# mikelodder7/bls-bn254

Hardware: AMD Instinct MI355X
Metric: BN254 pairings/sec (= BLS verifies/sec) (higher is better)
Workload: dtype int64; 1 GPU; 262144 batched single-sig BLS verifies per GPU (BASELINE configs[1]), unique 32-byte messages, 1024-key pool, 1/64 invalid tuples; key de-duplication + hash-to-G1 + per-key G2 checks and line tables + 2-pair Miller loop + final exp; tuples_per_gpu=262144, tuples_total=262144, key_pool=1024

## Files before the change

### bls-bn254_amd/csrc/pairing.h

```cpp
#pragma once
#include "curve.h"

namespace bn {

struct G2J { Fp2 x, y, z; };
struct Line { Fp2 c0, c1, c2; };

BN_FUNC Line doubling_step(G2J& r) {
  BN_CTX;
  Fp2 tmp0 = fp2_sqr(r.x);
  Fp2 tmp1 = fp2_sqr(r.y);
  Fp2 tmp2 = fp2_sqr(tmp1);
  Fp2 s3 = fp2_sqr(fp2_norm(fp2_add(tmp1, r.x)));
  Fp2 tmp3 = f_lc3<2, -2, -2>(s3, tmp0, tmp2);
  Fp2 tmp4 = f_lc2<3, 0>(tmp0, tmp0);
  Fp2 tmp6 = fp2_norm(fp2_add(r.x, tmp4));
  Fp2 tmp5 = fp2_sqr(tmp4);
  Fp2 zsq = fp2_sqr(r.z);
  Fp2 nx = f_lc2<1, -2>(tmp5, tmp3);
  Fp2 nz = fp2_norm(fp2_sub(fp2_sub(fp2_sqr(fp2_norm(fp2_add(r.z, r.y))), tmp1), zsq));
  Fp2 ny = f_lc2<1, -8>(fp2_mul(fp2_sub(tmp3, nx), tmp4), tmp2);
  Line l;
  l.c1 = f_lc2<-2, 0>(fp2_mul(tmp4, zsq), zsq);
  Fp2 s6 = fp2_sub(fp2_sub(fp2_sqr(tmp6), tmp0), tmp5);
  l.c2 = f_lc2<1, -4>(s6, tmp1);
  l.c0 = f_lc2<2, 0>(fp2_mul(nz, zsq), zsq);
  r.x = nx; r.y = ny; r.z = nz;
  return l;
}
BN_FUNC Line addition_step(G2J& r, const Fp2& qx, const Fp2& qy) {
  BN_CTX;
  Fp2 zsq = fp2_sqr(r.z);
  Fp2 ysq = fp2_sqr(qy);
  Fp2 t0 = fp2_mul(zsq, qx);
  Fp2 sy = fp2_sqr(fp2_norm(fp2_add(qy, r.z)));
  Fp2 t1 = fp2_mul(fp2_norm(fp2_sub(fp2_sub(sy, ysq), zsq)), zsq);
  Fp2 t2 = fp2_norm(fp2_sub(t0, r.x));
  Fp2 t3 = fp2_sqr(t2);
  Fp2 t4 = f_lc2<4, 0>(t3, t3);
  Fp2 t5 = fp2_mul(t4, t2);
  Fp2 t6 = f_lc2<1, -2>(t1, r.y);
  Fp2 t9 = fp2_mul(t6, qx);
  Fp2 t7 = fp2_mul(t4, r.x);
  Fp2 nx = f_lc3<1, -1, -2>(fp2_sqr(t6), t5, t7);
  Fp2 nz = fp2_norm(fp2_sub(fp2_sub(fp2_sqr(fp2_norm(fp2_add(r.z, t2))), zsq), t3));
  Fp2 t8 = fp2_mul(fp2_sub(t7, nx), t6);
  Fp2 ny = f_lc2<1, -2>(t8, fp2_mul(r.y, t5));
  Fp2 s10 = fp2_sqr(fp2_norm(fp2_add(qy, nz)));
  Fp2 t10 = fp2_sub(fp2_sub(s10, ysq), fp2_sqr(nz));
  Line l;
  l.c2 = f_lc2<2, -1>(t9, t10);
  l.c0 = f_lc2<2, 0>(nz, nz);
  l.c1 = f_lc2<-2, 0>(t6, t6);
  r.x = nx; r.y = ny; r.z = nz;
  return l;
}
BN_FUNC Fp12 ell(const Fp12& f, const Line& l, const Fp& px, const Fp& py) {
  BN_CTX;
  return fp12_mul_by_034(f, fp2_mul_fp(l.c0, py), fp2_mul_fp(l.c1, px), l.c2);
}
BN_FUNC Fp12 ell2(const Fp12& f, const Line& la, const Fp& pax, const Fp& pay, const Line& lb, const Fp& pbx, const Fp& pby) {
  BN_CTX;
  return fp12_mul_by_two_lines(f, fp2_mul_fp(la.c0, pay), fp2_mul_fp(la.c1, pax), la.c2, fp2_mul_fp(lb.c0, pby), fp2_mul_fp(lb.c1, pbx), lb.c2);
}
BN_INL Line fp2_norm_line(const Line& l) { return {fp2_norm(l.c0), fp2_norm(l.c1), fp2_norm(l.c2)}; }
BN_INL Line line_from_table(const int32_t* t) {
  return {fp2_from_limbs(t), fp2_from_limbs(t + 18), fp2_from_limbs(t + 36)};
}

constexpr uint64_t ate_naf_mask(int word, bool neg) {
  uint64_t m = 0;
  for (int i = 0; i < 64; ++i) {
    int j = 64 * word + i;
    if (j < bnc::ATE_NAF_LEN && (neg ? bnc::ATE_NAF[j] < 0 : bnc::ATE_NAF[j] != 0)) m |= (uint64_t)1 << i;
  }
  return m;
}
BN_INL int ate_naf_digit(int j) {
  constexpr uint64_t nz0 = ate_naf_mask(0, false), nz1 = ate_naf_mask(1, false), ng0 = ate_naf_mask(0, true), ng1 = ate_naf_mask(1, true);
  const uint64_t nz = j < 64 ? nz0 : nz1, ng = j < 64 ? ng0 : ng1;
  const int b = j & 63;
  return ((nz >> b) & 1) ? (((ng >> b) & 1) ? -1 : 1) : 0;
}
BN_FUNC Fp12 miller_loop_1(const G1A& p, const G2A& q) {
  BN_CTX;
  Fp12 f = fp12_one();
  G2J T = {q.x, q.y, fp2_one()};
  Fp2 nqy = fp2_norm(fp2_neg(q.y));
  for (int j = bnc::ATE_NAF_LEN - 2; j >= 0; --j) {
    f = fp12_sqr(f);
    f = ell(f, doubling_step(T), p.x, p.y);
    int d = ate_naf_digit(j);
    if (d != 0) f = ell(f, addition_step(T, q.x, d > 0 ? q.y : nqy), p.x, p.y);
  }
  Fp2 g2 = fp2_const(bnc::GAMMA1[1]), g3 = fp2_const(bnc::GAMMA1[2]);
  Fp2 q1x = fp2_mul(fp2_norm(fp2_conj(q.x)), g2), q1y = fp2_mul(fp2_norm(fp2_conj(q.y)), g3);
  Fp2 q2x = fp2_mul(fp2_norm(fp2_conj(q1x)), g2);
  Fp2 q2y = fp2_norm(fp2_neg(fp2_mul(fp2_norm(fp2_conj(q1y)), g3)));
  f = ell(f, addition_step(T, q1x, q1y), p.x, p.y);
  f = ell(f, addition_step(T, q2x, q2y), p.x, p.y);
  return f;
}

BN_FUNC Fp12 miller_loop_verify(const G1A& sig, const G1A& h, const G2A& pk,
                                     const int32_t (*table)[54]) {
  BN_CTX;
  Fp12 f = fp12_one();
  G2J T = {pk.x, pk.y, fp2_one()};
  Fp2 nqy = fp2_norm(fp2_neg(pk.y));
  int ti = 0;
  for (int j = bnc::ATE_NAF_LEN - 2; j >= 0; --j) {
    f = fp12_sqr(f);
    f = ell(f, line_from_table(table[ti++]), sig.x, sig.y);
    f = ell(f, doubling_step(T), h.x, h.y);
    int d = ate_naf_digit(j);
    if (d != 0) {
      f = ell(f, line_from_table(table[ti++]), sig.x, sig.y);
      f = ell(f, addition_step(T, pk.x, d > 0 ? pk.y : nqy), h.x, h.y);
    }
  }
  Fp2 g2 = fp2_const(bnc::GAMMA1[1]), g3 = fp2_const(bnc::GAMMA1[2]);
  Fp2 q1x = fp2_mul(fp2_norm(fp2_conj(pk.x)), g2), q1y = fp2_mul(fp2_norm(fp2_conj(pk.y)), g3);
  Fp2 q2x = fp2_mul(fp2_norm(fp2_conj(q1x)), g2);
  Fp2 q2y = fp2_norm(fp2_neg(fp2_mul(fp2_norm(fp2_conj(q1y)), g3)));
  f = ell(f, line_from_table(table[ti++]), sig.x, sig.y);
  f = ell(f, addition_step(T, q1x, q1y), h.x, h.y);
  f = ell(f, line_from_table(table[ti++]), sig.x, sig.y);
  f = ell(f, addition_step(T, q2x, q2y), h.x, h.y);
  return f;
}

BN_FUNC Fp12 miller_loop_verify_ws(const Ws& inv, const int32_t (*table)[54]) {
  Fp12 f = fp12_one();
  G2J T = {fp2_load_mem(ws_at(inv, 36)), fp2_load_mem(ws_at(inv, 54)), fp2_one()};
  int ti = 0;
  Ws p = inv;
  for (int j = bnc::ATE_NAF_LEN - 2; j >= 0; --j) {
    f = fp12_sqr(f);
    BN_OPAQUE(p);
    Fp sx = fp_load_mem(p), sy = fp_load_mem(ws_at(p, 9)), hx = fp_load_mem(ws_at(p, 18)), hy = fp_load_mem(ws_at(p, 27));
    BN_SCHED_BARRIER;
    Line l = doubling_step(T);
    f = ell2(f, line_from_table(table[ti++]), sx, sy, l, hx, hy);
    int d = ate_naf_digit(j);
    if (d != 0) {
      BN_OPAQUE(p);
      Fp2 qy = fp2_load_mem(ws_at(p, 54));
      Fp2 nqy = fp2_norm(fp2_neg(qy));
      Fp2 qx = fp2_load_mem(ws_at(p, 36));
      BN_OPAQUE(p);
      sx = fp_load_mem(p); sy = fp_load_mem(ws_at(p, 9)); hx = fp_load_mem(ws_at(p, 18)); hy = fp_load_mem(ws_at(p, 27));
      BN_SCHED_BARRIER;
      l = addition_step(T, qx, fp2_select(d > 0, qy, nqy));
      f = ell2(f, line_from_table(table[ti++]), sx, sy, l, hx, hy);
    }
  }
  BN_OPAQUE(p);
  Fp2 g2 = fp2_const(bnc::GAMMA1[1]), g3 = fp2_const(bnc::GAMMA1[2]);
  Fp2 q1x = fp2_mul(fp2_norm(fp2_conj(fp2_load_mem(ws_at(p, 36)))), g2);
  Fp2 q1y = fp2_mul(fp2_norm(fp2_conj(fp2_load_mem(ws_at(p, 54)))), g3);
  Fp2 q2x = fp2_mul(fp2_norm(fp2_conj(q1x)), g2);
  Fp2 q2y = fp2_norm(fp2_neg(fp2_mul(fp2_norm(fp2_conj(q1y)), g3)));
  Line l = addition_step(T, q1x, q1y);
  BN_OPAQUE(p);
  f = ell2(f, line_from_table(table[ti++]), fp_load_mem(p), fp_load_mem(ws_at(p, 9)), l, fp_load_mem(ws_at(p, 18)), fp_load_mem(ws_at(p, 27)));
  l = addition_step(T, q2x, q2y);
  BN_OPAQUE(p);
  f = ell2(f, line_from_table(table[ti++]), fp_load_mem(p), fp_load_mem(ws_at(p, 9)), l, fp_load_mem(ws_at(p, 18)), fp_load_mem(ws_at(p, 27)));
  return f;
}

BN_INL void g2j_store(const Ws& w, const G2J& t) { fp2_store_mem(w, t.x); fp2_store_mem(ws_at(w, 18), t.y); fp2_store_mem(ws_at(w, 36), t.z); }
BN_INL G2J g2j_load(const Ws& w) { return {fp2_load_mem(w), fp2_load_mem(ws_at(w, 18)), fp2_load_mem(ws_at(w, 36))}; }
BN_FUNC Fp12 miller_loop_verify_ws2(const Ws& inv, const Ws& park_in, const int32_t (*table)[54]) {
  Fp12 f = fp12_one();
  Ws p = inv, park = park_in;
  fp2_store_mem(park, fp2_load_mem(ws_at(inv, 36))); fp2_store_mem(ws_at(park, 18), fp2_load_mem(ws_at(inv, 54))); fp2_store_mem(ws_at(park, 36), fp2_one());
  BN_MEM_FENCE;
  int ti = 0;
  for (int j = bnc::ATE_NAF_LEN - 2; j >= 0; --j) {
    f = fp12_sqr(f);
    BN_OPAQUE(p); BN_OPAQUE(park);
    Fp sx = fp_load_mem(p), sy = fp_load_mem(ws_at(p, 9)), hx = fp_load_mem(ws_at(p, 18)), hy = fp_load_mem(ws_at(p, 27));
    G2J T = g2j_load(park);
    BN_SCHED_BARRIER;
    Line l = doubling_step(T);
    g2j_store(park, T);
    BN_MEM_FENCE;
    f = ell2(f, line_from_table(table[ti++]), sx, sy, l, hx, hy);
    int d = ate_naf_digit(j);
    if (d != 0) {
      BN_OPAQUE(p); BN_OPAQUE(park);
      Fp2 qy = fp2_load_mem(ws_at(p, 54));
      Fp2 nqy = fp2_norm(fp2_neg(qy));
      Fp2 qx = fp2_load_mem(ws_at(p, 36));
      sx = fp_load_mem(p); sy = fp_load_mem(ws_at(p, 9)); hx = fp_load_mem(ws_at(p, 18)); hy = fp_load_mem(ws_at(p, 27));
      T = g2j_load(park);
      BN_SCHED_BARRIER;
      l = addition_step(T, qx, fp2_select(d > 0, qy, nqy));
      g2j_store(park, T);
      BN_MEM_FENCE;
      f = ell2(f, line_from_table(table[ti++]), sx, sy, l, hx, hy);
    }
  }
  BN_OPAQUE(p); BN_OPAQUE(park);
  Fp2 g2 = fp2_const(bnc::GAMMA1[1]), g3 = fp2_const(bnc::GAMMA1[2]);
  Fp2 q1x = fp2_mul(fp2_norm(fp2_conj(fp2_load_mem(ws_at(p, 36)))), g2);
  Fp2 q1y = fp2_mul(fp2_norm(fp2_conj(fp2_load_mem(ws_at(p, 54)))), g3);
  Fp2 q2x = fp2_mul(fp2_norm(fp2_conj(q1x)), g2);
  Fp2 q2y = fp2_norm(fp2_neg(fp2_mul(fp2_norm(fp2_conj(q1y)), g3)));
  G2J T = g2j_load(park);
  Line l = addition_step(T, q1x, q1y);
  BN_OPAQUE(p);
  f = ell2(f, line_from_table(table[ti++]), fp_load_mem(p), fp_load_mem(ws_at(p, 9)), l, fp_load_mem(ws_at(p, 18)), fp_load_mem(ws_at(p, 27)));
  l = addition_step(T, q2x, q2y);
  BN_OPAQUE(p);
  f = ell2(f, line_from_table(table[ti++]), fp_load_mem(p), fp_load_mem(ws_at(p, 9)), l, fp_load_mem(ws_at(p, 18)), fp_load_mem(ws_at(p, 27)));
  return f;
}

BN_FUNC Fp12 miller_loop_1_ws(const Ws& inv_in, const Ws& park_in) {
  Fp12 f = fp12_one();
  Ws p = inv_in, park = park_in;
  fp2_store_mem(park, fp2_load_mem(ws_at(p, 18))); fp2_store_mem(ws_at(park, 18), fp2_load_mem(ws_at(p, 36))); fp2_store_mem(ws_at(park, 36), fp2_one());
  BN_MEM_FENCE;
  for (int j = bnc::ATE_NAF_LEN - 2; j >= 0; --j) {
    f = fp12_sqr(f);
    BN_OPAQUE(p); BN_OPAQUE(park);
    Fp px = fp_load_mem(p), py = fp_load_mem(ws_at(p, 9));
    G2J T = g2j_load(park);
    BN_SCHED_BARRIER;
    Line l = doubling_step(T);
    g2j_store(park, T);
    BN_MEM_FENCE;
    f = ell(f, l, px, py);
    int d = ate_naf_digit(j);
    if (d != 0) {
      BN_OPAQUE(p); BN_OPAQUE(park);
      Fp2 qy = fp2_load_mem(ws_at(p, 36));
      Fp2 nqy = fp2_norm(fp2_neg(qy));
      Fp2 qx = fp2_load_mem(ws_at(p, 18));
      px = fp_load_mem(p); py = fp_load_mem(ws_at(p, 9));
      T = g2j_load(park);
      BN_SCHED_BARRIER;
      l = addition_step(T, qx, fp2_select(d > 0, qy, nqy));
      g2j_store(park, T);
      BN_MEM_FENCE;
      f = ell(f, l, px, py);
    }
  }
  BN_OPAQUE(p); BN_OPAQUE(park);
  Fp2 g2 = fp2_const(bnc::GAMMA1[1]), g3 = fp2_const(bnc::GAMMA1[2]);
  Fp2 q1x = fp2_mul(fp2_norm(fp2_conj(fp2_load_mem(ws_at(p, 18)))), g2);
  Fp2 q1y = fp2_mul(fp2_norm(fp2_conj(fp2_load_mem(ws_at(p, 36)))), g3);
  Fp2 q2x = fp2_mul(fp2_norm(fp2_conj(q1x)), g2);
  Fp2 q2y = fp2_norm(fp2_neg(fp2_mul(fp2_norm(fp2_conj(q1y)), g3)));
  G2J T = g2j_load(park);
  Line l = addition_step(T, q1x, q1y);
  BN_OPAQUE(p);
  f = ell(f, l, fp_load_mem(p), fp_load_mem(ws_at(p, 9)));
  l = addition_step(T, q2x, q2y);
  BN_OPAQUE(p);
  f = ell(f, l, fp_load_mem(p), fp_load_mem(ws_at(p, 9)));
  return f;
}

BN_INL void line_store(const Ws& w, const Line& l) { fp2_store_mem(w, l.c0); fp2_store_mem(ws_at(w, 18), l.c1); fp2_store_mem(ws_at(w, 36), l.c2); }
BN_INL Line line_load(const Ws& w) { return {fp2_load_mem(w), fp2_load_mem(ws_at(w, 18)), fp2_load_mem(ws_at(w, 36))}; }
BN_INL Line line_mask(bool live, const Line& l) {
  return {fp2_select(live, l.c0, fp2_one()), fp2_select(live, l.c1, fp2_zero()), fp2_select(live, l.c2, fp2_zero())};
}
template <int KIND>
BN_FUNC Fp12 miller2_step(const Fp12& f_in, G2J& T, const Ws& park, const Ws& lpark, const Ws& hh_in, const Ws& qw_in, bool negq, bool live_a, bool live_b) {
  Ws hh = hh_in, qw = qw_in, pk = park, lp = lpark;
  BN_OPAQUE(hh); BN_OPAQUE(qw); BN_OPAQUE(pk); BN_OPAQUE(lp);
  const Fp2 g2 = fp2_const(bnc::GAMMA1[1]), g3 = fp2_const(bnc::GAMMA1[2]);
  auto q_of = [&](int pair, Fp2& qx, Fp2& qy) {
    qx = fp2_load_mem(ws_at(qw, 36 * pair)); qy = fp2_load_mem(ws_at(qw, 36 * pair + 18));
    if (KIND == 1) qy = fp2_select(negq, fp2_norm(fp2_neg(qy)), qy);
    if (KIND >= 2) { qx = fp2_mul(fp2_norm(fp2_conj(qx)), g2); qy = fp2_mul(fp2_norm(fp2_conj(qy)), g3); }
    if (KIND == 3) { qx = fp2_mul(fp2_norm(fp2_conj(qx)), g2); qy = fp2_norm(fp2_neg(fp2_mul(fp2_norm(fp2_conj(qy)), g3))); }
  };
  Line la;
  if (KIND == 0) la = doubling_step(T);
  else { Fp2 qx, qy; q_of(0, qx, qy); la = addition_step(T, qx, qy); }
  line_store(lp, fp2_norm_line(line_mask(live_a, la)));
  G2J Tb = g2j_load(pk);
  BN_MEM_FENCE;
  g2j_store(pk, T);
  BN_MEM_FENCE;
  Line lb;
  if (KIND == 0) lb = doubling_step(Tb);
  else { Fp2 qx, qy; q_of(1, qx, qy); lb = addition_step(Tb, qx, qy); }
  lb = line_mask(live_b, lb);
  T = g2j_load(pk);
  BN_MEM_FENCE;
  g2j_store(pk, Tb);
  BN_MEM_FENCE;
  la = line_load(lp);
  Fp hax = fp_load_mem(hh), hay = fp_load_mem(ws_at(hh, 9)), hbx = fp_load_mem(ws_at(hh, 18)), hby = fp_load_mem(ws_at(hh, 27));
  return ell2(f_in, la, hax, hay, lb, hbx, hby);
}
BN_FUNC Fp12 miller_loop_2var_ws(const Ws& hh, const Ws& qw, const Ws& park, const Ws& lpark, bool live_a, bool live_b) {
  Fp12 f = fp12_one();
  G2J T = {fp2_load_mem(qw), fp2_load_mem(ws_at(qw, 18)), fp2_one()};
  g2j_store(park, G2J{fp2_load_mem(ws_at(qw, 36)), fp2_load_mem(ws_at(qw, 54)), fp2_one()});
  BN_MEM_FENCE;
  for (int j = bnc::ATE_NAF_LEN - 2; j >= 0; --j) {
    f = fp12_sqr(f);
    f = miller2_step<0>(f, T, park, lpark, hh, qw, false, live_a, live_b);
    int d = ate_naf_digit(j);
    if (d != 0) f = miller2_step<1>(f, T, park, lpark, hh, qw, d < 0, live_a, live_b);
  }
  f = miller2_step<2>(f, T, park, lpark, hh, qw, false, live_a, live_b);
  f = miller2_step<3>(f, T, park, lpark, hh, qw, false, live_a, live_b);
  return f;
}

BN_FUNC Fp12 cyclotomic_exp_x(const Fp12& f) {
  BN_CTX;
  Fp12 r = f;
  for (int i = 61; i >= 0; --i) {
    r = fp12_cyclotomic_sqr(r);
    if ((bnc::BN_X >> i) & 1) r = fp12_mul(r, f);
  }
  return r;
}
BN_FUNC Fp12 cyclotomic_exp_x_chain(const Fp12& f, const Ws& slots, const Ws* park = nullptr) {
  const ChainOp prog[BN_X_CHAIN_LEN] = BN_X_CHAIN;
  fp12_store_mem(slots, f);
  BN_MEM_FENCE;
  Fp12 r = f;
  for (int k = 0; k < BN_X_CHAIN_LEN; ++k) {
    const ChainOp op = prog[k];
    if (op.load >= 0) r = fp12_load_mem(ws_at(slots, 108 * op.load));
    for (int q = 0; q < op.sq; ++q) r = fp12_cyclotomic_sqr(r);
    if (op.mul >= 0) r = fp12_mul_mem(r, ws_at(slots, 108 * op.mul), park);
    if (op.store >= 0) fp12_store_mem(ws_at(slots, 108 * op.store), r);
    if (op.cstore >= 0) { fp6_store_mem(ws_at(slots, 108 * op.cstore), r.c0); fp6_store_mem(ws_at(slots, 108 * op.cstore + 54), fp6_norm(fp6_neg(r.c1))); }
    if (op.store >= 0 || op.cstore >= 0) BN_MEM_FENCE;
  }
  return r;
}
BN_FUNC Fp12 fe_easy(const Fp12& f) {
  Fp12 t = fp12_mul(fp12_conj(f), fp12_inv(f));
  return fp12_mul(fp12_frob<2>(t), t);
}
struct FeEasyHead { Fp2 c0, c1, c2, nrm; Fp nu; };
BN_FUNC FeEasyHead fe_easy_head(const Fp12& a) {
  BN_CTX;
  Fp6 s0 = fp6_sqr(a.c0), s1 = fp6_sqr(a.c1);
  Fp6 d = {fp2_sub_mul_xi(s0.c0, s1.c2), fp2_norm(fp2_sub(s0.c1, s1.c0)), fp2_norm(fp2_sub(s0.c2, s1.c1))};
  Fp2 q0 = fp2_sqr(d.c0), q1 = fp2_sqr(d.c1), q2 = fp2_sqr(d.c2);
  Fp2 m01 = fp2_mul(d.c0, d.c1), m02 = fp2_mul(d.c0, d.c2), m12 = fp2_mul(d.c1, d.c2);
  FeEasyHead h;
  h.c0 = fp2_sub_mul_xi(q0, m12);
  h.c1 = fp2_norm(fp2_sub(fp2_mul_xi(q2), m01));
  h.c2 = fp2_norm(fp2_sub(q1, m02));
  Fp2 u = fp2_add(fp2_mul(d.c2, h.c1), fp2_mul(d.c1, h.c2));
  h.nrm = fp2_add_mul_xi(fp2_mul(d.c0, h.c0), u);
  h.nu = fp_dot2(h.nrm.c0, h.nrm.c0, h.nrm.c1, h.nrm.c1);
  return h;
}
BN_FUNC Fp12 fe_easy_tail(const Fp12& a, const FeEasyHead& h, const Fp& nu_inv) {
  BN_CTX;
  Fp2 ti = {fp_mul(h.nrm.c0, nu_inv), fp_mul(fp_neg(h.nrm.c1), nu_inv)};
  Fp6 t6 = {fp2_mul(h.c0, ti), fp2_mul(h.c1, ti), fp2_mul(h.c2, ti)};
  Fp12 inv = {fp6_mul(a.c0, t6), fp6_norm(fp6_neg(fp6_mul(a.c1, t6)))};
  Fp12 t = fp12_mul(fp12_conj(a), inv);
  return fp12_mul(fp12_frob<2>(t), t);
}
template <bool POW_FALLBACK = true>
BN_FUNC bool fp_inv4(Fp x[4]) {
  BN_CTX;
  bool z[4];
  Fp v[4], pre[4];
  for (int i = 0; i < 4; ++i) { z[i] = fp_is_zero(x[i]); v[i] = fp_select(z[i], fp_one(), fp_norm(x[i])); }
  pre[0] = v[0];
  for (int i = 1; i < 4; ++i) pre[i] = fp_mul(pre[i - 1], v[i]);
  bool done = true;
  Fp inv = POW_FALLBACK ? fp_inv(pre[3]) : fp_inv_divsteps(pre[3], done);
  for (int i = 3; i >= 1; --i) {
    Fp r = fp_mul(inv, pre[i - 1]);
    inv = fp_mul(inv, v[i]);
    x[i] = fp_select(z[i], fp_zero(), r);
  }
  x[0] = fp_select(z[0], fp_zero(), inv);
  return done;
}
BN_FUNC void fe_h1(const Fp12& x0, Fp12& a, Fp12& b) {
  a = fp12_cyclotomic_sqr(fp12_conj(x0));
  Fp12 a2 = fp12_cyclotomic_sqr(a);
  b = fp12_mul(a, a2);
}
BN_FUNC void fe_h2(const Fp12& x0, const Fp12& b, Fp12& c, Fp12& b2, Fp12& d2) {
  c = fp12_conj(x0);
  b2 = fp12_mul(c, fp12_conj(b));
  d2 = fp12_cyclotomic_sqr(c);
}
BN_FUNC Fp12 fe_h3(const Fp12& t, const Fp12& a, const Fp12& c, const Fp12& b2, const Fp12& x0) {
  Fp12 e = fp12_mul(b2, x0);
  Fp12 d = fp12_mul(a, e);
  Fp12 l0 = fp12_mul(t, fp12_mul(c, e));
  Fp12 r = fp12_mul(l0, fp12_frob<1>(d));
  r = fp12_mul(r, fp12_frob<2>(e));
  Fp12 l3 = fp12_mul(fp12_conj(t), d);
  return fp12_mul(r, fp12_frob<3>(l3));
}
BN_FUNC Fp12 final_exponentiation(const Fp12& f) {
  Fp12 t = fe_easy(f), a, b, c, b2, d2;
  fe_h1(cyclotomic_exp_x(t), a, b);
  fe_h2(cyclotomic_exp_x(b), b, c, b2, d2);
  return fe_h3(t, a, c, b2, cyclotomic_exp_x(d2));
}

BN_INL void fp2_to_be(uint8_t* out, const Fp2& c) { fp_to_be(out, c.c0); fp_to_be(out + 32, c.c1); }
BN_FUNC void fp12_to_be(uint8_t* out, const Fp12& a) {
  BN_CTX;
  fp2_to_be(out, a.c0.c0); fp2_to_be(out + 64, a.c0.c1); fp2_to_be(out + 128, a.c0.c2);
  fp2_to_be(out + 192, a.c1.c0); fp2_to_be(out + 256, a.c1.c1); fp2_to_be(out + 320, a.c1.c2);
}
BN_INL Fp2 fp2_from_be(const uint8_t* in, bool& ok) {
  bool o0, o1;
  Fp2 c = {fp_from_be(in, o0), fp_from_be(in + 32, o1)};
  ok &= o0 & o1;
  return c;
}
BN_FUNC Fp12 fp12_from_be(const uint8_t* in, bool& ok) {
  BN_CTX;
  ok = true;
  Fp12 a;
  a.c0.c0 = fp2_from_be(in, ok); a.c0.c1 = fp2_from_be(in + 64, ok); a.c0.c2 = fp2_from_be(in + 128, ok);
  a.c1.c0 = fp2_from_be(in + 192, ok); a.c1.c1 = fp2_from_be(in + 256, ok); a.c1.c2 = fp2_from_be(in + 320, ok);
  return a;
}
BN_INL void fp2_store_limbs(int32_t* out, size_t stride, const Fp2& c) {
  Fp c0 = fp_canon(c.c0), c1 = fp_canon(c.c1);
  BN_UNROLL for (int k = 0; k < NL; ++k) { out[(size_t)k * stride] = c0.l[k]; out[(size_t)(9 + k) * stride] = c1.l[k]; }
}
BN_INL void fp2_store_limbs(const Ws& w, const Fp2& c) {
  Fp c0 = fp_canon(c.c0), c1 = fp_canon(c.c1);
  BN_UNROLL for (int k = 0; k < NL; ++k) { ws_store(w, k, c0.l[k]); ws_store(w, 9 + k, c1.l[k]); }
}
BN_FUNC void fp12_store_limbs(const Ws& w, const Fp12& a) {
  BN_CTX;
  fp2_store_limbs(w, a.c0.c0); fp2_store_limbs(ws_at(w, 18), a.c0.c1); fp2_store_limbs(ws_at(w, 36), a.c0.c2);
  fp2_store_limbs(ws_at(w, 54), a.c1.c0); fp2_store_limbs(ws_at(w, 72), a.c1.c1); fp2_store_limbs(ws_at(w, 90), a.c1.c2);
}
BN_INL Fp2 fp2_load_limbs(const Ws& w) {
  Fp2 c;
  BN_UNROLL for (int k = 0; k < NL; ++k) { c.c0.l[k] = ws_load(w, k); c.c1.l[k] = ws_load(w, 9 + k); }
  BN_TRK(set_trk(c.c0, 0, 1, 0, 0.006, 1); set_trk(c.c1, 0, 1, 0, 0.006, 1);)
  return c;
}
BN_FUNC Fp12 fp12_load_limbs(const Ws& w) {
  BN_CTX;
  return {{fp2_load_limbs(w), fp2_load_limbs(ws_at(w, 18)), fp2_load_limbs(ws_at(w, 36))},
          {fp2_load_limbs(ws_at(w, 54)), fp2_load_limbs(ws_at(w, 72)), fp2_load_limbs(ws_at(w, 90))}};
}
BN_FUNC void fp12_store_limbs(int32_t* out, size_t stride, const Fp12& a) {
  BN_CTX;
  fp2_store_limbs(out, stride, a.c0.c0); fp2_store_limbs(out + 18 * stride, stride, a.c0.c1);
  fp2_store_limbs(out + 36 * stride, stride, a.c0.c2); fp2_store_limbs(out + 54 * stride, stride, a.c1.c0);
  fp2_store_limbs(out + 72 * stride, stride, a.c1.c1); fp2_store_limbs(out + 90 * stride, stride, a.c1.c2);
}
BN_INL Fp2 fp2_load_limbs(const int32_t* in, size_t stride) {
  Fp2 c;
  BN_UNROLL for (int k = 0; k < NL; ++k) { c.c0.l[k] = in[(size_t)k * stride]; c.c1.l[k] = in[(size_t)(9 + k) * stride]; }
  BN_TRK(set_trk(c.c0, 0, 1, 0, 0.006, 1); set_trk(c.c1, 0, 1, 0, 0.006, 1);)
  return c;
}
BN_FUNC Fp12 fp12_load_limbs(const int32_t* in, size_t stride) {
  BN_CTX;
  return {{fp2_load_limbs(in, stride), fp2_load_limbs(in + 18 * stride, stride), fp2_load_limbs(in + 36 * stride, stride)},
          {fp2_load_limbs(in + 54 * stride, stride), fp2_load_limbs(in + 72 * stride, stride), fp2_load_limbs(in + 90 * stride, stride)}};
}

struct H3Op { int8_t pre, mul, post; };
BN_FUNC Fp12 fe_h3_loop(const Ws* src, const Ws& tmp, const Ws* park) {
  const H3Op prog[8] = {{1, 4, 1}, {0, 1, 2}, {2, 0, 3}, {3, 2, 0}, {0, 0, 0}, {0, 7, 0}, {0, 6, 0}, {0, 8, 0}};
  Fp12 r = fp12_one();
  for (int k = 0; k < 8; ++k) {
    const H3Op op = prog[k];
    if (op.pre == 1) r = fp12_load_mem(src[3]);
    else if (op.pre == 2) r = fp12_conj(r);
    else if (op.pre == 3) r = fp12_load_mem(tmp);
    const int m = op.mul;
    const Ws b = m == 0 ? src[0] : m == 1 ? src[1] : m == 2 ? src[2] : m == 4 ? src[4] : ws_at(tmp, 108 * (size_t)(m - 5));
    r = fp12_mul_mem(r, b, park);
    if (op.post == 1) { fp12_store_mem(tmp, r); fp12_store_mem(ws_at(tmp, 108), fp12_frob<2>(r)); }
    else if (op.post == 2) fp12_store_mem(ws_at(tmp, 216), fp12_frob<1>(r));
    else if (op.post == 3) fp12_store_mem(ws_at(tmp, 324), fp12_frob<3>(fp12_conj(r)));
    BN_MEM_FENCE;
  }
  return r;
}

BN_FUNC void fe_h1_tail(const Fp12& x0, const Ws& a_out, const Ws& b_out, const Ws* park) {
  Fp12 a = fp12_cyclotomic_sqr(fp12_conj(x0));
  fp12_store_mem(a_out, a);
  BN_MEM_FENCE;
  fp12_store_mem(b_out, fp12_mul_mem(fp12_cyclotomic_sqr(a), a_out, park));
}
BN_FUNC void fe_h2_tail(const Fp12& x0, const Ws& b_in, const Ws& c_out, const Ws& b2_out, const Ws& d2_out, const Ws* park) {
  fp12_store_mem(c_out, fp12_conj(x0));
  BN_MEM_FENCE;
  fp12_store_mem(b2_out, fp12_conj(fp12_mul_mem(x0, b_in, park)));
  BN_MEM_FENCE;
  fp12_store_mem(d2_out, fp12_cyclotomic_sqr(fp12_load_mem(c_out)));
}

BN_INL void line_store_limbs(const Ws& w, const Line& l) { fp2_store_limbs(w, l.c0); fp2_store_limbs(ws_at(w, 18), l.c1); fp2_store_limbs(ws_at(w, 36), l.c2); }
BN_INL Line line_load_limbs(const Ws& w) { return {fp2_load_limbs(w), fp2_load_limbs(ws_at(w, 18)), fp2_load_limbs(ws_at(w, 36))}; }
BN_FUNC void g2_prepare_lines(const G2A& q, const Ws& out) {
  BN_CTX;
  G2J T = {q.x, q.y, fp2_one()};
  Fp2 nqy = fp2_norm(fp2_neg(q.y));
  int ti = 0;
  for (int j = bnc::ATE_NAF_LEN - 2; j >= 0; --j) {
    line_store_limbs(ws_at(out, 54 * (size_t)ti++), doubling_step(T));
    int d = ate_naf_digit(j);
    if (d != 0) line_store_limbs(ws_at(out, 54 * (size_t)ti++), addition_step(T, q.x, d > 0 ? q.y : nqy));
  }
  Fp2 g2 = fp2_const(bnc::GAMMA1[1]), g3 = fp2_const(bnc::GAMMA1[2]);
  Fp2 q1x = fp2_mul(fp2_norm(fp2_conj(q.x)), g2), q1y = fp2_mul(fp2_norm(fp2_conj(q.y)), g3);
  Fp2 q2x = fp2_mul(fp2_norm(fp2_conj(q1x)), g2);
  Fp2 q2y = fp2_norm(fp2_neg(fp2_mul(fp2_norm(fp2_conj(q1y)), g3)));
  line_store_limbs(ws_at(out, 54 * (size_t)ti++), addition_step(T, q1x, q1y));
  line_store_limbs(ws_at(out, 54 * (size_t)ti++), addition_step(T, q2x, q2y));
}
BN_INL void fp_store_limbs_lazy(const Ws& w, const Fp& c) {
  BN_TRK(if (c.lo < -4e-6 || c.hi > 1.0 + 4e-6 || c.tlo < -0.02 || c.thi > 0.02 || c.vb > 1.2) check_fail("pair table entry outside its declared range", c.vb);)
  BN_UNROLL for (int k = 0; k < NL; ++k) ws_store(w, k, c.l[k]);
}
BN_INL Fp fp_load_limbs_lazy(const Ws& w) {
  Fp c;
  BN_UNROLL for (int k = 0; k < NL; ++k) c.l[k] = ws_load(w, k);
  BN_TRK(set_trk(c, -4e-6, 1.0 + 4e-6, -0.02, 0.02, 1.2); check_actual(c, "pair table entry");)
  return c;
}
BN_INL void fp2_store_limbs_lazy(const Ws& w, const Fp2& c) { fp_store_limbs_lazy(w, c.c0); fp_store_limbs_lazy(ws_at(w, 9), c.c1); }
BN_INL Fp2 fp2_load_limbs_lazy(const Ws& w) {
  Fp2 c;
  BN_UNROLL for (int k = 0; k < NL; ++k) { c.c0.l[k] = ws_load(w, k); c.c1.l[k] = ws_load(w, 9 + k); }
  BN_TRK(set_trk(c.c0, -4e-6, 1.0 + 4e-6, -0.02, 0.02, 1.2); set_trk(c.c1, -4e-6, 1.0 + 4e-6, -0.02, 0.02, 1.2);
         check_actual(c.c0, "pair table entry"); check_actual(c.c1, "pair table entry");)
  return c;
}
BN_FUNC void line_pair_expand(const Line& a, const Line& b, const Ws& out) {
  BN_CTX;
  fp2_store_limbs_lazy(out, fp2_mul(a.c0, b.c0));
  fp2_store_limbs_lazy(ws_at(out, 18), fp2_mul_xi(fp2_mul(a.c2, b.c2)));
  fp2_store_limbs_lazy(ws_at(out, 36), fp2_mul(a.c1, b.c1));
  fp2_store_limbs_lazy(ws_at(out, 54), fp2_mul(a.c1, b.c2));
  fp2_store_limbs_lazy(ws_at(out, 72), fp2_mul(a.c2, b.c1));
  fp2_store_limbs_lazy(ws_at(out, 90), fp2_mul(a.c0, b.c1));
  fp2_store_limbs_lazy(ws_at(out, 108), fp2_mul(a.c1, b.c0));
  fp2_store_limbs_lazy(ws_at(out, 126), fp2_mul(a.c0, b.c2));
  fp2_store_limbs_lazy(ws_at(out, 144), fp2_mul(a.c2, b.c0));
}
BN_INL Fp2 fp2_dot_fp(const Fp2& t, const Fp& s, const Fp2& u, const Fp& r) {
  return {fp_dot2(t.c0, s, u.c0, r), fp_dot2(t.c1, s, u.c1, r)};
}
BN_FUNC Fp12 ell_pair_expanded(const Fp12& f, const Ws& e, const Ws& cw) {
  BN_CTX;
  Fp X = fp_load_mem(cw), Y = fp_load_mem(ws_at(cw, 9)), Z = fp_load_mem(ws_at(cw, 18));
  Fp xsX = fp_load_mem(ws_at(cw, 27)), ysY = fp_load_mem(ws_at(cw, 36)), xsZ = fp_load_mem(ws_at(cw, 45));
  Fp ysZ = fp_load_mem(ws_at(cw, 54)), ysX = fp_load_mem(ws_at(cw, 63)), xsY = fp_load_mem(ws_at(cw, 72));
  Fp6 l0 = {fp2_dot_fp(fp2_load_limbs_lazy(e), ysY, fp2_load_limbs_lazy(ws_at(e, 18)), Z),
            fp2_mul_fp(fp2_load_limbs_lazy(ws_at(e, 36)), xsX),
            fp2_dot_fp(fp2_load_limbs_lazy(ws_at(e, 54)), xsZ, fp2_load_limbs_lazy(ws_at(e, 72)), X)};
  Fp2 l10 = fp2_dot_fp(fp2_load_limbs_lazy(ws_at(e, 90)), ysX, fp2_load_limbs_lazy(ws_at(e, 108)), xsY);
  Fp2 l11 = fp2_dot_fp(fp2_load_limbs_lazy(ws_at(e, 126)), ysZ, fp2_load_limbs_lazy(ws_at(e, 144)), Y);
  Fp6 v0 = fp6_mul(f.c0, l0);
  Fp6 v1 = fp6_mul_by_01(f.c1, l10, l11);
  Fp6 dl = {fp2_norm(fp2_sub(l10, l0.c0)), fp2_norm(fp2_sub(l11, l0.c1)), fp2_norm(fp2_neg(l0.c2))};
  Fp6 w = fp6_mul(fp6_norm(fp6_sub(f.c0, f.c1)), dl);
  return {fp6_add_mul_v(v0, v1), fp6_norm(fp6_add(fp6_add(w, v0), v1))};
}
BN_FUNC Fp12 miller_loop_prepared(const Ws& inv, const Ws& ktab_in) {
  Fp12 f = fp12_one();
  Ws p = inv, kt = ktab_in;
  int ti = 0;
  for (int j = bnc::ATE_NAF_LEN - 2; j >= 0; --j) {
    f = fp12_sqr(f);
    BN_OPAQUE(kt); BN_OPAQUE(p);
    f = ell_pair_expanded(f, ws_at(kt, 162 * (size_t)ti), p);
    ++ti;
    if (ate_naf_digit(j) != 0) {
      BN_OPAQUE(kt); BN_OPAQUE(p);
      f = ell_pair_expanded(f, ws_at(kt, 162 * (size_t)ti), p);
      ++ti;
    }
  }
  for (int e = 0; e < 2; ++e) {
    BN_OPAQUE(kt); BN_OPAQUE(p);
    f = ell_pair_expanded(f, ws_at(kt, 162 * (size_t)ti), p);
    ++ti;
  }
  return f;
}
BN_FUNC void fp2_inv4(Fp2 x[4], bool zero[4]) {
  BN_CTX;
  Fp2 n[4];
  Fp nu[4];
  for (int i = 0; i < 4; ++i) { n[i] = fp2_norm(x[i]); nu[i] = fp_dot2(n[i].c0, n[i].c0, n[i].c1, n[i].c1); }
  const bool done = fp_inv4<false>(nu);
  for (int i = 0; i < 4; ++i) {
    zero[i] = !done | fp_is_zero(nu[i]);
    x[i] = {fp_mul(n[i].c0, nu[i]), fp_mul(fp_neg(n[i].c1), nu[i])};
  }
}
BN_INL Fp2 fp2_unit_line_const(const int32_t* c) {
  Fp2 r;
  BN_UNROLL for (int i = 0; i < NL; ++i) { r.c0.l[i] = c[i]; r.c1.l[i] = c[NL + i]; }
  BN_TRK(set_trk(r.c0, 0, 1, 0, 0.006, 1); set_trk(r.c1, 0, 1, 0, 0.006, 1);)
  return r;
}
struct UnitPair { Fp2 a0, a4, u0, u4; };
BN_FUNC UnitPair unit_pair_of(const int32_t* au, const Fp2& b0, const Fp2& b3_inv, const Fp2& b4) {
  BN_CTX;
  return {fp2_unit_line_const(au), fp2_unit_line_const(au + 18), fp2_mul(b0, b3_inv), fp2_mul(b4, b3_inv)};
}
BN_INL Fp2 unit_pair_entry(const UnitPair& q, int j) {
  return j == 0 ? fp2_mul(q.a0, q.u0) : j == 1 ? fp2_mul_xi(fp2_mul(q.a4, q.u4)) : j == 2 ? fp2_one() : j == 3 ? q.u4 : j == 4 ? q.a4
       : j == 5 ? q.a0 : j == 6 ? q.u0 : j == 7 ? fp2_mul(q.a0, q.u4) : fp2_mul(q.a4, q.u0);
}
BN_FUNC void line_pair_expand_unit(const int32_t* au, const Fp2& b0, const Fp2& b3_inv, const Fp2& b4, const Ws& out) {
  BN_CTX;
  const UnitPair q = unit_pair_of(au, b0, b3_inv, b4);
  for (int j = 0; j < 9; ++j) fp2_store_limbs_lazy(ws_at(out, 18 * (size_t)j), unit_pair_entry(q, j));
}
BN_FUNC bool miller_unit_coords(const Fp& xs, const Fp& ys, const Fp& X, const Fp& Y, const Fp& Z, const Ws& cw, bool& ok) {
  BN_CTX;
  const Fp xsX = fp_mul(xs, X);
  const bool unit = !fp_is_zero(xsX);
  const Fp s = fp_select(unit, fp_inv_divsteps(xsX, ok), fp_one());
  const Fp Xs = fp_mul(X, s), Ys = fp_mul(Y, s), Zs = fp_mul(Z, s);
  fp_store_mem(cw, Ys); fp_store_mem(ws_at(cw, 9), Zs);
  fp_store_mem(ws_at(cw, 18), fp_mul(ys, Ys)); fp_store_mem(ws_at(cw, 27), fp_mul(xs, Zs)); fp_store_mem(ws_at(cw, 36), fp_mul(ys, Zs));
  fp_store_mem(ws_at(cw, 45), fp_mul(ys, Xs)); fp_store_mem(ws_at(cw, 54), fp_mul(xs, Ys)); fp_store_mem(ws_at(cw, 63), Xs);
  return unit;
}
BN_FUNC Fp6 fp6_mul_unit1(const Fp6& a, const Fp2& b0, const Fp2& b2, bool unit) {
  BN_CTX;
  const Fp2 b1 = fp2_select(unit, fp2_one(), fp2_zero());
  Fp2 v0 = fp2_mul(a.c0, b0), v1 = fp2_select(unit, a.c1, fp2_zero()), v2 = fp2_mul(a.c2, b2);
  Fp2 w0 = fp2_mul(fp2_sub(a.c1, a.c2), fp2_sub(b1, b2));
  Fp2 w1 = fp2_mul(fp2_sub(a.c0, a.c1), fp2_sub(b0, b1));
  Fp2 w2 = fp2_mul(fp2_sub(a.c0, a.c2), fp2_sub(b0, b2));
  Fp2 t0 = fp2_sub(fp2_add(v1, v2), w0);
  Fp2 t1 = fp2_sub(fp2_add(v0, v1), w1);
  Fp2 t2 = fp2_sub(fp2_add(v0, v2), w2);
  return {fp2_add_mul_xi(v0, t0), fp2_add_mul_xi(t1, v2), fp2_norm(fp2_add(t2, v1))};
}
BN_FUNC Fp12 ell_pair_unit(const Fp12& f, const Ws& e, const Ws& cw, bool unit) {
  BN_CTX;
  Fp Y = fp_load_mem(cw), Z = fp_load_mem(ws_at(cw, 9)), ysY = fp_load_mem(ws_at(cw, 18)), xsZ = fp_load_mem(ws_at(cw, 27));
  Fp ysZ = fp_load_mem(ws_at(cw, 36)), ysX = fp_load_mem(ws_at(cw, 45)), xsY = fp_load_mem(ws_at(cw, 54)), X = fp_load_mem(ws_at(cw, 63));
  Fp2 l00 = fp2_dot_fp(fp2_load_limbs_lazy(e), ysY, fp2_load_limbs_lazy(ws_at(e, 18)), Z);
  Fp2 l02 = fp2_dot_fp(fp2_load_limbs_lazy(ws_at(e, 54)), xsZ, fp2_load_limbs_lazy(ws_at(e, 72)), X);
  Fp2 l10 = fp2_dot_fp(fp2_load_limbs_lazy(ws_at(e, 90)), ysX, fp2_load_limbs_lazy(ws_at(e, 108)), xsY);
  Fp2 l11 = fp2_dot_fp(fp2_load_limbs_lazy(ws_at(e, 126)), ysZ, fp2_load_limbs_lazy(ws_at(e, 144)), Y);
  Fp6 v0 = fp6_mul_unit1(f.c0, l00, l02, unit);
  Fp6 v1 = fp6_mul_by_01(f.c1, l10, l11);
  Fp6 dl = {fp2_norm(fp2_sub(l10, l00)), fp2_norm(fp2_sub(l11, fp2_select(unit, fp2_one(), fp2_zero()))), fp2_norm(fp2_neg(l02))};
  Fp6 w = fp6_mul(fp6_norm(fp6_sub(f.c0, f.c1)), dl);
  return {fp6_add_mul_v(v0, v1), fp6_norm(fp6_add(fp6_add(w, v0), v1))};
}
BN_FUNC Fp12 miller_loop_prepared_unit(const Ws& cw, const Ws& ktab_in, bool unit) {
  Fp12 f = fp12_one();
  Ws p = cw, kt = ktab_in;
  int ti = 0;
  for (int j = bnc::ATE_NAF_LEN - 2; j >= 0; --j) {
    f = fp12_sqr(f);
    BN_OPAQUE(kt); BN_OPAQUE(p);
    f = ell_pair_unit(f, ws_at(kt, 162 * (size_t)ti), p, unit);
    ++ti;
    if (ate_naf_digit(j) != 0) {
      BN_OPAQUE(kt); BN_OPAQUE(p);
      f = ell_pair_unit(f, ws_at(kt, 162 * (size_t)ti), p, unit);
      ++ti;
    }
  }
  for (int e = 0; e < 2; ++e) {
    BN_OPAQUE(kt); BN_OPAQUE(p);
    f = ell_pair_unit(f, ws_at(kt, 162 * (size_t)ti), p, unit);
    ++ti;
  }
  return f;
}

BN_FUNC Fp12 miller_loop_1prepared(const Ws& hh_in, const Ws& ta_in) {
  Fp12 f = fp12_one();
  Ws hh = hh_in, ta = ta_in;
  int ti = 0;
  for (int j = bnc::ATE_NAF_LEN - 2; j >= 0; --j) {
    f = fp12_sqr(f);
    BN_OPAQUE(ta); BN_OPAQUE(hh);
    f = ell(f, line_load_limbs(ws_at(ta, 54 * (size_t)ti)), fp_load_mem(hh), fp_load_mem(ws_at(hh, 9)));
    ++ti;
    if (ate_naf_digit(j) != 0) {
      BN_OPAQUE(ta); BN_OPAQUE(hh);
      f = ell(f, line_load_limbs(ws_at(ta, 54 * (size_t)ti)), fp_load_mem(hh), fp_load_mem(ws_at(hh, 9)));
      ++ti;
    }
  }
  for (int e = 0; e < 2; ++e) {
    BN_OPAQUE(ta); BN_OPAQUE(hh);
    f = ell(f, line_load_limbs(ws_at(ta, 54 * (size_t)ti)), fp_load_mem(hh), fp_load_mem(ws_at(hh, 9)));
    ++ti;
  }
  return f;
}

BN_FUNC Fp12 ell2_from_tables(const Fp12& f, const Ws& ta_in, const Ws& tb_in, int ti, const Ws& hh_in, bool live_a, bool live_b) {
  Ws hh = hh_in, ta = ta_in, tb = tb_in;
  BN_OPAQUE(ta); BN_OPAQUE(tb); BN_OPAQUE(hh);
  Line la = line_mask(live_a, line_load_limbs(ws_at(ta, 54 * (size_t)ti)));
  Line lb = line_mask(live_b, line_load_limbs(ws_at(tb, 54 * (size_t)ti)));
  Fp hax = fp_load_mem(hh), hay = fp_load_mem(ws_at(hh, 9)), hbx = fp_load_mem(ws_at(hh, 18)), hby = fp_load_mem(ws_at(hh, 27));
  return ell2(f, la, hax, hay, lb, hbx, hby);
}
BN_FUNC Fp12 miller_loop_2prepared(const Ws& hh, const Ws& ta, const Ws& tb, bool live_a, bool live_b) {
  Fp12 f = fp12_one();
  int ti = 0;
  for (int j = bnc::ATE_NAF_LEN - 2; j >= 0; --j) {
    f = fp12_sqr(f);
    f = ell2_from_tables(f, ta, tb, ti++, hh, live_a, live_b);
    if (ate_naf_digit(j) != 0) f = ell2_from_tables(f, ta, tb, ti++, hh, live_a, live_b);
  }
  f = ell2_from_tables(f, ta, tb, ti++, hh, live_a, live_b);
  f = ell2_from_tables(f, ta, tb, ti++, hh, live_a, live_b);
  return f;
}

}
```

Before: 7.372 million verifies/s.

## Rewrite sparse line multiplication with interpolation-based Fp12 product formulas

Replaces the Karatsuba-style sparse Fp12-by-line multiply in the Miller loop (a unit-coefficient Fp6 multiply, a sparse 01 multiply and a full Fp6 cross term) with a hand-derived evaluation/interpolation scheme. It computes products at points ±1 and combines them with lazy linear combinations, aiming to cut the number of Fp2 multiplications and reductions per line evaluation. Scheduling barriers are placed between stages to limit register pressure. The risk is more additions and linear-combination work, and possible correctness errors in the derived coefficients.

Result: faster. 7.853 million verifies/s, median of 6 (+6.5%).

```diff
diff --git a/bls-bn254_amd/csrc/pairing.h b/bls-bn254_amd/csrc/pairing.h
--- a/bls-bn254_amd/csrc/pairing.h
+++ b/bls-bn254_amd/csrc/pairing.h
@@ -642,31 +642,59 @@
   fp_store_mem(ws_at(cw, 45), fp_mul(ys, Xs)); fp_store_mem(ws_at(cw, 54), fp_mul(xs, Ys)); fp_store_mem(ws_at(cw, 63), Xs);
   return unit;
 }
-BN_FUNC Fp6 fp6_mul_unit1(const Fp6& a, const Fp2& b0, const Fp2& b2, bool unit) {
-  BN_CTX;
-  const Fp2 b1 = fp2_select(unit, fp2_one(), fp2_zero());
-  Fp2 v0 = fp2_mul(a.c0, b0), v1 = fp2_select(unit, a.c1, fp2_zero()), v2 = fp2_mul(a.c2, b2);
-  Fp2 w0 = fp2_mul(fp2_sub(a.c1, a.c2), fp2_sub(b1, b2));
-  Fp2 w1 = fp2_mul(fp2_sub(a.c0, a.c1), fp2_sub(b0, b1));
-  Fp2 w2 = fp2_mul(fp2_sub(a.c0, a.c2), fp2_sub(b0, b2));
-  Fp2 t0 = fp2_sub(fp2_add(v1, v2), w0);
-  Fp2 t1 = fp2_sub(fp2_add(v0, v1), w1);
-  Fp2 t2 = fp2_sub(fp2_add(v0, v2), w2);
-  return {fp2_add_mul_xi(v0, t0), fp2_add_mul_xi(t1, v2), fp2_norm(fp2_add(t2, v1))};
-}
+template <int K1, int K2, int K3, int K4>
+BN_INL Fp fp_lc4r(const Fp& x1, const Fp& x2, const Fp& x3, const Fp& x4) { return fp_lc4<K1, K2, K3, K4, true>(x1, x2, x3, x4); }
 BN_FUNC Fp12 ell_pair_unit(const Fp12& f, const Ws& e, const Ws& cw, bool unit) {
   BN_CTX;
   Fp Y = fp_load_mem(cw), Z = fp_load_mem(ws_at(cw, 9)), ysY = fp_load_mem(ws_at(cw, 18)), xsZ = fp_load_mem(ws_at(cw, 27));
   Fp ysZ = fp_load_mem(ws_at(cw, 36)), ysX = fp_load_mem(ws_at(cw, 45)), xsY = fp_load_mem(ws_at(cw, 54)), X = fp_load_mem(ws_at(cw, 63));
-  Fp2 l00 = fp2_dot_fp(fp2_load_limbs_lazy(e), ysY, fp2_load_limbs_lazy(ws_at(e, 18)), Z);
-  Fp2 l02 = fp2_dot_fp(fp2_load_limbs_lazy(ws_at(e, 54)), xsZ, fp2_load_limbs_lazy(ws_at(e, 72)), X);
-  Fp2 l10 = fp2_dot_fp(fp2_load_limbs_lazy(ws_at(e, 90)), ysX, fp2_load_limbs_lazy(ws_at(e, 108)), xsY);
-  Fp2 l11 = fp2_dot_fp(fp2_load_limbs_lazy(ws_at(e, 126)), ysZ, fp2_load_limbs_lazy(ws_at(e, 144)), Y);
-  Fp6 v0 = fp6_mul_unit1(f.c0, l00, l02, unit);
-  Fp6 v1 = fp6_mul_by_01(f.c1, l10, l11);
-  Fp6 dl = {fp2_norm(fp2_sub(l10, l00)), fp2_norm(fp2_sub(l11, fp2_select(unit, fp2_one(), fp2_zero()))), fp2_norm(fp2_neg(l02))};
-  Fp6 w = fp6_mul(fp6_norm(fp6_sub(f.c0, f.c1)), dl);
-  return {fp6_add_mul_v(v0, v1), fp6_norm(fp6_add(fp6_add(w, v0), v1))};
+  const Fp2 l0 = fp2_dot_fp(fp2_load_limbs_lazy(e), ysY, fp2_load_limbs_lazy(ws_at(e, 18)), Z);
+  const Fp2 l4 = fp2_dot_fp(fp2_load_limbs_lazy(ws_at(e, 54)), xsZ, fp2_load_limbs_lazy(ws_at(e, 72)), X);
+  const Fp2 l1 = fp2_dot_fp(fp2_load_limbs_lazy(ws_at(e, 90)), ysX, fp2_load_limbs_lazy(ws_at(e, 108)), xsY);
+  const Fp2 l3 = fp2_dot_fp(fp2_load_limbs_lazy(ws_at(e, 126)), ysZ, fp2_load_limbs_lazy(ws_at(e, 144)), Y);
+  const Fp2 &g0 = f.c0.c0, &g2 = f.c0.c1, &g4 = f.c0.c2, &g1 = f.c1.c0, &g3 = f.c1.c1, &g5 = f.c1.c2;
+  const Fp2 sa = fp2_add(g0, g2);
+  Fp2 e1 = fp2_norm(fp2_add(sa, g1)), em = fp2_norm(fp2_sub(sa, g1));
+  Fp2 h1 = fp2_norm(fp2_add(l0, l1)), hm = fp2_sub(l0, l1);
+  const Fp2 A0 = fp2_mul(g0, l0), Ai = fp2_mul(g2, l1);
+  Fp2 Ap, Ad;
+  { const Fp2 m1 = fp2_mul(e1, h1), mm = fp2_mul(em, hm); Ap = fp2_add(m1, mm); Ad = fp2_sub(m1, mm); }
+  BN_SCHED_BARRIER;
+  const Fp2 sb = fp2_add(g3, g5);
+  const Fp2 B0 = fp2_mul(g3, l3), Bi = fp2_mul(g5, l4);
+  Fp2 Bp, Bd;
+  { const Fp2 k1 = fp2_norm(fp2_add(sb, g4)), n1 = fp2_norm(fp2_add(l3, l4));
+    const Fp2 m1 = fp2_mul(k1, n1);
+    e1 = fp2_sub(e1, k1); h1 = fp2_sub(h1, n1);
+    const Fp2 km = fp2_norm(fp2_sub(sb, g4)), nm = fp2_sub(l3, l4);
+    const Fp2 mm = fp2_mul(km, nm);
+    em = fp2_sub(em, km); hm = fp2_norm(fp2_sub(hm, nm));
+    Bp = fp2_add(m1, mm); Bd = fp2_sub(m1, mm); }
+  Fp2 Cp, Cd;
+  { const Fp2 m1 = fp2_mul(e1, h1), mm = fp2_mul(em, hm); Cp = fp2_add(m1, mm); Cd = fp2_sub(m1, mm); }
+  const Fp2 C0 = fp2_mul(fp2_sub(g0, g3), fp2_sub(l0, l3)), Ci = fp2_mul(fp2_sub(g2, g5), fp2_sub(l1, l4));
+  BN_SCHED_BARRIER;
+  const Fp2 T0 = fp2_sub(fp2_add(A0, B0), C0), Ti = fp2_sub(fp2_add(Ai, Bi), Ci);
+  const Fp2 z = fp2_zero();
+  Fp12 r;
+  { const Fp2 u2 = fp2_select(unit, g2, z), u5 = fp2_select(unit, g5, z);
+    const Fp2 d = fp2_sub(fp2_add(Ad, Bd), Cd), t = fp2_sub(Ti, u2);
+    r.c0.c2 = {fp_lc4r<1, -2, 0, 0>(d.c0, t.c0, d.c0, d.c0), fp_lc4r<1, -2, 0, 0>(d.c1, t.c1, d.c1, d.c1)};
+    const Fp2 x = fp2_sub(Ad, fp2_dbl(Ai)), y = fp2_add(Bd, fp2_dbl(fp2_sub(u5, Bi)));
+    r.c1.c0 = fp2_add_mul_xi(x, y); }
+  BN_SCHED_BARRIER;
+  { const Fp2 u0 = fp2_select(unit, g0, z), u3 = fp2_select(unit, g3, z);
+    const Fp2 p = fp2_sub(Ap, Cp), t = fp2_sub(T0, u3);
+    r.c1.c2 = {fp_lc4r<1, 1, -2, 0>(p.c0, Bp.c0, t.c0, p.c0), fp_lc4r<1, 1, -2, 0>(p.c1, Bp.c1, t.c1, p.c1)};
+    const Fp2 s = fp2_sub(u0, A0), y = fp2_sub(Bp, fp2_dbl(B0));
+    r.c0.c1 = {fp_lc4<1, 2, 9, -1>(Ap.c0, s.c0, y.c0, y.c1), fp_lc4<1, 2, 1, 9>(Ap.c1, s.c1, y.c0, y.c1)}; }
+  BN_SCHED_BARRIER;
+  { const Fp2 u1 = fp2_select(unit, g1, z), u4 = fp2_select(unit, g4, z);
+    const Fp2 x = fp2_add(Ai, u1);
+    r.c1.c1 = {fp_lc4<2, 2, 18, -2>(x.c0, T0.c0, Bi.c0, Bi.c1), fp_lc4<2, 2, 2, 18>(x.c1, T0.c1, Bi.c0, Bi.c1)};
+    const Fp2 y = fp2_add(B0, Ti);
+    r.c0.c0 = {fp_lc4<2, 18, -2, 18>(fp_sub(A0.c0, u4.c1), y.c0, y.c1, u4.c0), fp_lc4<2, 2, 18, 18>(fp_add(A0.c1, u4.c0), y.c0, y.c1, u4.c1)}; }
+  return r;
 }
 BN_FUNC Fp12 miller_loop_prepared_unit(const Ws& cw, const Ws& ktab_in, bool unit) {
   Fp12 f = fp12_one();
```
